# ykevinc/pocket-tts

Measured on AMD Instinct MI355X. Metric: audio-sec/wall-sec (RTF) per GPU at batch=32 + p50 first-chunk latency, higher is better.
Workload: dtype f32; 1 GPU; b6369a24 batch=32 concurrent 10 s utterances per GPU (125 frames, voice prompt 125 frames, 40 text tokens), lsd_decode_steps=1 (BASELINE configs[2]); global_batch=32, utterance_frames=125, jobs=37, prompt_frames=125, parallelism=replicas x1

## Files before the change

### pocket-tts_amd/csrc/engine.cpp

```cpp
#include "engine.h"

#include <hip/hip_ext.h>

#include <algorithm>
#include <array>
#include <cstdlib>
#include <cmath>
#include <cstring>
#include <mutex>

namespace ptts {

namespace {
std::mutex& voice_mu() {
  static std::mutex m;
  return m;
}

int pick_splits(int M, int N, int K) {
  const int tiles = ((N + 31) / 32) * ((M + 31) / 32);
  const int chunks = K / 32;
  int s = std::max(1, 768 / std::max(1, tiles));
  s = std::min(s, std::max(1, chunks / 4));
  return std::min(s, 16);
// ... 164 lines not shown
  vpre_ = (const float**)dalloc((sizeof(float*) * B + 3) / 4);
  vlen_ = (int*)dalloc(B);
  slot_voice_.assign(B, nullptr);
  drained_.assign(B, 1);
  codec_ok_.assign(B, 1);
  admit_call_.assign(B, -1);
  slot_lsd_.assign(B, 0);
  cancelled_.assign(B, 0);
  share_voice_ = probe_env("PTTS_NO_SHARED_VOICE") == nullptr;
  if (share_voice_) {
    fbm_.kv.pre = vpre_;
    fbm_.kv.pre_len = vlen_;
  }
#ifdef PTTS_PROBES
  if (probe_env("PTTS_STAMPS")) {
    stamp_ring_ = (unsigned long long*)dalloc((size_t)STAMP_CAP * 4);
    stamp_ctr_ = (unsigned*)dalloc(1);
  }
#endif
  if (probe_env("PTTS_BACK_WG_CAP")) back_cap_ = atoi(probe_env("PTTS_BACK_WG_CAP"));
  if (probe_env("PTTS_FRONT_PRIO")) set_front_prio(atoi(probe_env("PTTS_FRONT_PRIO")));
  if (probe_env("PTTS_BACK_PRIO")) set_back_prio(atoi(probe_env("PTTS_BACK_PRIO")));
  if (probe_env("PTTS_FRONT_SKIP")) set_front_skip(atoi(probe_env("PTTS_FRONT_SKIP")));
  ysilu_ = dalloc((size_t)lsd_ * B * FD);
  mods_ = dalloc((size_t)lsd_ * B * NADA);
  xf_ = dalloc((size_t)B * FD);
  hf_ = dalloc((size_t)B * FD);
  uf_ = dalloc((size_t)B * FD);
  PTTS_REQUIRE(hx_floats(B) * 4 < (1ull << 31), "flow-head hand-off regions exceed 2 GB (lsd_decode_steps too large)");
  hx_ = dalloc(hx_floats(B));
  fhm_ = dalloc((size_t)lsd_ * ((B + 15) / 16) * (FDEPTH + 1) * 2 * 16 * FD);
  PTTS_HIP(hipMemset(hx_, 0xFF, hx_floats(B) * 4));
  PTTS_HIP(hipDeviceSynchronize());
  hctr_ = (int*)dalloc(4 * ((B + 15) / 16) + 4);
  herr_ = (int*)dalloc(4);
  for (int i = 0, ch = MD / 2; i < 3; ++i, ch /= 2) trb_[i] = dalloc((size_t)RATIOS[i] * ch);
  temb_ =dalloc((size_t)temb_row0(lsd_ + 1) * FD);
  rope_ = dalloc((size_t)max_ctx_ * 64);
  temb_tmp_ = dalloc((size_t)2 * lsd_ * FD);

  for (int q = 0; q < NHB; ++q) {
    h_pcm_[q] = (float*)halloc(sizeof(float) * B * FRAME);
    h_meta_[q] = nfr_ > 1 && q < nhb_ ? h_pcmp_[q / nfr_] + (size_t)B * nfr_ * FRAME + (q % nfr_) * mstride
                                      : (float*)halloc(sizeof(float) * meta_floats_);
    memset(h_meta_[q], 0, sizeof(float) * meta_floats_);
  }
  h_err_ = (int*)halloc(sizeof(int));
  *h_err_ = 0;
  h_slots_ = (int*)halloc(sizeof(int) * B);
  h_st_ = (SlotState*)halloc(sizeof(SlotState) * B);
  h_idle_ = (SlotState*)halloc(sizeof(SlotState));
  *h_idle_ = SlotState{};
  h_idle_->eos_step = -1;
  h_fp_ = (int*)halloc(sizeof(int) * B);
  h_ids_ = (int*)halloc(sizeof(int) * PREFILL);
  h_tab_ = (int*)halloc(sizeof(int) * 4 * PREFILL);
  h_plat_ = (float*)halloc(sizeof(float) * PREFILL * LDIM);
  h_alat_ = (float*)halloc(sizeof(float) * B * LDIM);
  h_aopt_ = (int*)halloc(sizeof(int) * B);
  h_vpre_ = (const float**)halloc(sizeof(const float*) * B);
  h_vlen_ = (int*)halloc(sizeof(int) * B);
  memset(h_vpre_, 0, sizeof(float*) * B);
  memset(h_vlen_, 0, sizeof(int) * B);
  PTTS_HIP(hipStreamCreateWithFlags(&stream_be_, hipStreamNonBlocking));
  for (int q = 0; q < NHB; ++q) {
    PTTS_HIP(hipEventCreateWithFlags(&ev_front_[q], hipEventDisableTiming));
// ... 240 lines not shown
  auto it = split_.find(a.W);
  PTTS_REQUIRE(it != split_.end(), "bf16x6 tile without a split weight copy");
  a.Whm = it->second.first;
  a.Wlo = it->second.second;
}

void Engine::finalize() {
  PTTS_HIP(hipSetDevice(dev_));
  if (wq_ != QUANT_NONE && q8map_.empty()) derive_int8();
  if (fp8_ && f8map_.empty()) derive_fp8();
  if (gvmap_.empty()) derive_gemv();
  if (back_mfma_ == PTTS_BACK_F32X6 && split_.empty()) derive_split();
  if (!inw_t_) {
    void* p = nullptr;
    PTTS_HIP(hipMalloc(&p, sizeof(float) * LDIM * D));
    allocs_.push_back(p);
    inw_t_ = (float*)p;
  }
  transpose(W(L_.input_linear), D, LDIM, inw_t_, stream_);
  if (!fh_inw_t_) {
    void* p = nullptr;
    PTTS_HIP(hipMalloc(&p, sizeof(float) * LDIM * FD));
    allocs_.push_back(p);
    fh_inw_t_ = (float*)p;
  }
  transpose(W(L_.inproj_w), FD, LDIM, fh_inw_t_, stream_);
  if (!fhw_ && head_uniform_stride()) {
    void* p = nullptr;
    PTTS_HIP(hipMalloc(&p, sizeof(float) * flow_head_packed_floats()));
    allocs_.push_back(p);
    fhw_ = (float*)p;
  }
  if (fhw_) pack_flow_head(W(L_.rb_w0[0]), W(L_.rb_w2[0]), (long)(L_.rb_w0[1] - L_.rb_w0[0]), W(L_.fin_w), fhw_, stream_);
  TimeEmbedWeights tw;
  for (int i = 0; i < 2; ++i) {
    tw.l1w[i] = W(L_.te_l1w[i]);
    tw.l1b[i] = W(L_.te_l1b[i]);
    tw.l2w[i] = W(L_.te_l2w[i]);
    tw.l2b[i] = W(L_.te_l2b[i]);
    tw.alpha[i] = W(L_.te_alpha[i]);
  }
  for (int n = 1; n <= lsd_; ++n) time_embeddings(tw, n, temb_tmp_, temb_ + (size_t)temb_row0(n) * FD, stream_);
  rope_table(rope_, max_ctx_, stream_);
  for (int i = 0, ch = MD / 2; i < 3; ++i, ch /= 2)
    for (int p = 0; p < RATIOS[i]; ++p)
      PTTS_HIP(hipMemcpyAsync(trb_[i] + (size_t)p * ch, W(L_.dtr_b[i]), sizeof(float) * ch, hipMemcpyDeviceToDevice,
                              stream_));
  PTTS_HIP(hipGetLastError());
  PTTS_HIP(hipStreamSynchronize(stream_));
  ready_ = true;
}

void Engine::run_ops(const std::vector<Op>& ops) {
  xh_dirty_ = true;
  run_ops_on(ops, stream_);
}

void Engine::run_ops_on(const std::vector<Op>& ops, hipStream_t s) {
  for (const Op& op : ops) {
    op.fn(s);
    hipError_t e = hipGetLastError();
    if (e != hipSuccess) throw Error(PTTS_ERR_HIP, "launch of " + op.name + " failed: " + hipGetErrorString(e));
  }
}

void Engine::derive_int8() {
// ... 233 lines not shown
    const Layout::TL& t = L_.fl[l];
    const std::string p = tag + ".l" + std::to_string(l);
    KvStore kv = fb.kv;
    kv.base += (long)l * fb.kv_layer;
    if (kv.pre) kv.layer = l;
    int S = 1;
    linear_split(ops, p + ".qkv_gemm", fb.h, D, M, W(t.in_proj), 3 * D, D, &S, fb);
    if (step) {
      const float* P = fb.partial;
      float* O = fb.o;
      const float* rope = rope_;
      const double L = plan_ctx_ > 0 ? plan_ctx_ : max_ctx_ / 2.0;
      const double kvu = plan_kvu_ > 0 ? plan_kvu_ : M * L;
      ops.push_back({p + ".attention", [=](hipStream_t s) { attention_step_qkv(P, S, M, NH, map, kv, rope, O, s); },
                     (double)M * 4096.0 * L,
                     8192.0 * kvu + (double)M * (4.0 * (S * 3.0 * D + 2.0 * D + D) + 64.0 * 4 * 2)});
    } else {
      {
        const float* P = fb.partial;
        float* Q = fb.q;
        ops.push_back({p + ".qkv_rope", [=](hipStream_t s) { qkv_rope_append(P, S, nullptr, M, NH, map, kv, Q, s); }});
      }
      const float* Q = fb.q;
      float* O = fb.o;
      RowMap am = map;
      int Ma = M;
      if (map.ptab) {
        am.tab = map.ptab;
        Ma = map.mpad;
      }
      ops.push_back({p + ".attention", [=](hipStream_t s) { attention(Q, Ma, NH, am, kv, 0, O, s); }});
    }
    auto rr = [&](const std::string& name, int S2, int N, int act, bool resid, float* Y, const float* lnw,
                  const float* lnb, bool ln, float* Hout, float* Hfrag = nullptr) {
      RowReduceArgs a{};
      a.Hfrag = Hfrag;
      a.P = fb.partial;
      a.S = S2;
      a.M = M;
      a.N = N;
      a.act = act;
      if (resid) {
        a.R = fb.x;
        a.ldr = D;
      }
      a.Y = Y;
      a.ldy = N;
      a.ln = ln ? 1 : 0;
      a.ln_w = lnw;
      a.ln_b = lnb;
      a.eps = 1e-5f;
      a.Hout = Hout;
      a.ldh = N;
      push_rr(ops, name, a);
    };
    linear_split(ops, p + ".out_gemm", fb.o, D, M, W(t.out_proj), D, D, &S, fb);
    auto fk = step && gemv_fk_supported(M, FF, D) ? fkmap_.find(W(t.l1)) : fkmap_.end();
    const bool use_fk = fk != fkmap_.end() && hfrag_;
    rr(p + ".out_reduce_ln2", S, D, ACT_NONE, true, fb.x, W(t.n2w), W(t.n2b), true, fb.h, use_fk ? hfrag_ : nullptr);
    auto ffn = use_fk && ffn_hand_ ? ffnmap_.find(W(t.l2)) : ffnmap_.end();
    if (ffn != ffnmap_.end()) {
      static_assert(NL % 2 == 0, "the fused FFN's hand-off sets alternate by layer");
      const float *A = hfrag_, *P1 = fk->second, *P2 = ffn->second;
      float *hand = ffn_hand_, *Pp = fb.partial;
      int* err = herr_;
      const int set = l & 1;
      const int groups = ffn_groups_;
      auto f8 = ffn8map_.find(W(t.l2));
      const uint32_t *Q1 = nullptr, *Q2 = nullptr;
      const float *s1 = nullptr, *s2 = nullptr;
      if (f8 != ffn8map_.end()) {
        Q1 = f8->second.first.first;
        s1 = f8->second.first.second;
        Q2 = f8->second.second.first;
        s2 = f8->second.second.second;
      }
      const bool e4m3 = fp8_ && Q1;
      Op op{p + ".ffn", [=](hipStream_t s) { ffn_fused(A, M, P1, P2, groups, hand, set, Pp, err, s, Q1, s1, Q2, s2, e4m3); },
            2.0 * M * FF * D * 2,
            (Q1 ? 2.0 * FF * D + 8.0 * (FF + D) : 8.0 * FF * D) + 4.0 * ((double)M * D + (double)groups * M * D)};
      op.prep = [hand](hipStream_t s) { PTTS_HIP(hipMemsetD32Async(hand, 0xFFFFFFFFu, 2 * FFN_HAND_FLOATS, s)); };
      ops.push_back(op);
      S = groups;
    } else {
      if (use_fk) {
        const float* Pk = fk->second;
        const float* A = hfrag_;
        float* U = fb.u;
        ops.push_back({p + ".ff1_gemm", [=](hipStream_t s) { gemv_fk(A, M, FF, Pk, nullptr, ACT_GELU, U, FF, s); },
                       2.0 * M * FF * D, 4.0 * ((double)FF * D + (double)M * D + (double)M * FF)});
      } else {
        linear_split(ops, p + ".ff1_gemm", fb.h, D, M, W(t.l1), FF, D, &S, fb);
        rr(p + ".ff1_reduce_gelu", S, FF, ACT_GELU, false, fb.u, nullptr, nullptr, false, nullptr);
      }
      linear_split(ops, p + ".ff2_gemm", fb.u, FF, M, W(t.l2), D, FF, &S, fb);
    }
    if (l + 1 < NL)
      rr(p + ".ff2_reduce_ln1", S, D, ACT_NONE, true, fb.x, W(L_.fl[l + 1].n1w), W(L_.fl[l + 1].n1b), true, fb.h);
    else
      rr(p + ".ff2_reduce_outnorm", S, D, ACT_NONE, true, fb.x, W(L_.out_norm_w), W(L_.out_norm_b), out_norm, fb.h);
  }
}

void Engine::prefill_rows(std::vector<Op>& ops, int slot, int T, int p0, const FlowBufs& fb) {
  {
    float *x = fb.x, *h = fb.h;
    const float* w = W(L_.fl[0].n1w);
    const float* b = W(L_.fl[0].n1b);
    ops.push_back({"prefill.ln1", [=](hipStream_t s) { layernorm(x, D, h, D, T, D, w, b, 1e-5f, s); }});
  }
  RowMap map{slot, T, p0, nullptr};
  flow_layers(ops, T, map, false, false, "prefill", fb);
}

bool Engine::use_head_chain(int B) const {
  if (!flow_head_fits(B)) return false;
  if (flow_head_grid(B) > head_resident_) return false;
  return head_uniform_stride();
}

bool Engine::head_uniform_stride() const {
  const long s = (long)(L_.rb_w0[1] - L_.rb_w0[0]);
  for (int i = 1; i < FDEPTH; ++i)
    if ((long)(L_.rb_lnw[i] - L_.rb_lnw[i - 1]) != s || (long)(L_.rb_lnb[i] - L_.rb_lnb[i - 1]) != s ||
        (long)(L_.rb_w0[i] - L_.rb_w0[i - 1]) != s || (long)(L_.rb_b0[i] - L_.rb_b0[i - 1]) != s ||
        (long)(L_.rb_w2[i] - L_.rb_w2[i - 1]) != s || (long)(L_.rb_b2[i] - L_.rb_b2[i - 1]) != s)
      return false;
  return true;
}

void Engine::build_front(std::vector<Op>& ops, int B, int hb, int lsd_run) {
  PTTS_REQUIRE(lsd_run >= 1 && lsd_run <= lsd_, "lsd_run outside [1, cap]");
  int S = 1;
  const FlowBufs& fb = fbm_;
  flow_layers(ops, B, RowMap{0, 1, 0, fpos_}, true, true, "flow", fb);
  linear_split(ops, "head.cond_eos_gemm", fb.h, D, B, W(L_.cond_eos_w), NCOND, D, &S, fb);
  PTTS_REQUIRE(S <= FLOW_COND_MAX_SLABS, "head.flow_cond sums at most 16 split-K slabs");
  {
    const float* P = fb.partial;
    const float* bias = W(L_.cond_eos_b);
    const float* temb = temb_;
    const int lsd = lsd_run, cap = lsd_;
    SlotState* st = st_;
    float *ys = ysilu_, *cur = cur_, *eos = eos_;
    ops.push_back({"head.flow_cond", [=](hipStream_t s) { flow_cond(P, S, B, bias, temb, lsd, cap, st, ys, cur, eos, s); },
                   (double)B * NCOND * (S + 1) + 4.0 * lsd * B * FD,
                   4.0 * ((double)S * B * NCOND + NCOND + lsd * FD + lsd * (double)B * FD + B * (LDIM + 1.0))});
  }
  linear_split(ops, "head.ada_gemm", ysilu_, FD, lsd_run * B, W(L_.ada_w), NADA, FD, &S, fb);
  {
    RowReduceArgs a{};
    a.P = fb.partial;
    a.S = S;
    a.M = lsd_run * B;
    a.N = NADA;
    a.bias = W(L_.ada_b);
    a.Y = mods_;
    a.ldy = NADA;
    if (use_head_chain(B)) {
      const size_t r0 = (size_t)((B + 15) / 16 * 16) * FD;
      a.fill = hx_ + r0;
      a.fill_n4 = (long)((hx_floats(B, lsd_run) - r0) / 4);
      a.x0_cur = cur_;
      a.x0_w = fh_inw_t_;
      a.x0_b = W(L_.inproj_b);
      a.x0_hx = hx_;
      a.x0_B = B;
      a.fhm = fhm_;
      a.fhm_B = B;
    }
    push_rr(ops, "head.ada_reduce", a);
  }
  if (use_head_chain(B)) {
    FlowHeadArgs f{};
    f.B = B;
    f.lsd = lsd_run;
    f.st = st_;
    f.cur = cur_;
    f.mods = mods_;
    f.ldm = NADA;
    f.in_w = W(L_.inproj_w);
    f.in_b = W(L_.inproj_b);
    f.lnw = W(L_.rb_lnw[0]);
    f.lnb = W(L_.rb_lnb[0]);
    f.w0 = W(L_.rb_w0[0]);
    f.b0 = W(L_.rb_b0[0]);
    f.w2 = W(L_.rb_w2[0]);
    f.b2 = W(L_.rb_b2[0]);
    f.blk = (long)(L_.rb_w0[1] - L_.rb_w0[0]);
    f.fin_w = W(L_.fin_w);
    f.fin_b = W(L_.fin_b);
    f.wp = fhw_;
    f.fhm = fhm_;
    f.hx = hx_;
    f.x0_ready = 1;
    f.ctr = hctr_;
    f.err = herr_;
    f.dbg = probe_env("PTTS_HEAD_DBG") ? (unsigned long long*)strtoull(probe_env("PTTS_HEAD_DBG"), nullptr, 0) : nullptr;
    const double fl = 2.0 * lsd_run * B * ((double)FD * LDIM + 2.0 * FDEPTH * FD * FD + (double)LDIM * FD);
    const double by = 4.0 * ((double)FD * LDIM + 2.0 * FDEPTH * FD * FD + (double)LDIM * FD) +
                      4.0 * lsd_run * B * ((double)FDEPTH * 3 * FD + 2 * FD);
    float* hx = hx_;
    const size_t nhx = hx_floats(B, lsd_run);
    const float *cur = cur_, *iw = fh_inw_t_, *ib = W(L_.inproj_b);
// ... 2404 lines not shown
```

### pocket-tts_amd/csrc/engine.h

```cpp
#pragma once
#include <functional>
#include <map>
#include <string>
#include <vector>

#include "common.h"
#include "kernels.h"
#include "weights.h"

struct ptts_voice {
  int F = 0;
  float* kv = nullptr;
  std::vector<float> cond;
  const void* owner = nullptr;
  mutable int refs = 0;
  mutable bool dead = false;
  hipEvent_t ev = nullptr;
  float* h_cond = nullptr;
  mutable bool ordered = false;
};

namespace ptts {

struct VoicePlan;
// ... 175 lines not shown
  long ring_slot_ = 0, ring_layer_ = 0;
  int* fpos_ = nullptr;
  bool share_voice_ = true;
  const float** vpre_ = nullptr;
  int* vlen_ = nullptr;
  const float** h_vpre_ = nullptr;
  int* h_vlen_ = nullptr;
  std::vector<const ptts_voice*> slot_voice_;
  void voice_release(int slot, bool drained);
  SlotState* st_ = nullptr;
  float *lat_in_ = nullptr, *cur_ = nullptr, *eos_ = nullptr;
  int hist_T_[8] = {}, hist_C_[8] = {}, hist_P_[8] = {};

  static constexpr int PREFILL = 2048;
  static constexpr size_t TAIL_CAP = (size_t)16 << 20;
  static constexpr int TICKETS = 1024;
  int* ids_dev_ = nullptr;
  int* rowtab_dev_ = nullptr;
  int *ctab_dev_ = nullptr, *qrow_dev_ = nullptr, *orow_dev_ = nullptr;
  int* admit_slots_ = nullptr;
  SlotState* admit_st_ = nullptr;
  int* admit_fpos_ = nullptr;
  float *plat_dev_ = nullptr, *h_plat_ = nullptr, *admit_lat_ = nullptr, *h_alat_ = nullptr;
  int *admit_opt_ = nullptr, *h_aopt_ = nullptr;
  float *ysilu_ = nullptr, *mods_ = nullptr, *xf_ = nullptr, *hf_ = nullptr, *uf_ = nullptr;
  bool head_uniform_stride() const;
  bool use_head_chain(int B) const;
  float* fhw_ = nullptr;
  float* hx_ = nullptr;
  float* fhm_ = nullptr;
  float* fh_inw_t_ = nullptr;
  size_t hx_floats(int B) const { return hx_floats(B, lsd_); }
  size_t hx_floats(int B, int lsd) const { return (size_t)lsd * 13 * ((B + 15) / 16 * 16) * FD; }
  float* inw_t_ = nullptr;
  int *hctr_ = nullptr, *herr_ = nullptr;
  float* trb_[3] = {};
  static constexpr int NHB = NHB_MAX;
  int nhb_ = 3;
  int nfr_ = 1;
  int back_mfma_ = PTTS_BACK_F32;
  std::map<const float*, std::pair<const unsigned*, const unsigned short*>> split_;
  void derive_split();
  void attach_split(GemmArgs& a) const;
  int rows_hb_[NHB] = {};
  float* pcmp_[NHB / 2] = {};
  float* h_pcmp_[NHB / 2] = {};
  SlotState* h_act_ = nullptr;
  std::vector<int> act_slots_;
  int admit_delay_ = 0;
  double plan_ctx_ = 0, plan_win_ = 0, plan_kvu_ = 0;
  float* lat_out_[NHB] = {};
  float* eos_out_[NHB] = {};
  FrameFlags* flags_[NHB] = {};
  float* pcm_[NHB] = {};
  float* meta_[NHB] = {};
  size_t meta_floats_ = 0;
  int back_cap_ = 1;
  bool pipeline_ = false;
  hipStream_t stream_be_ = nullptr;
  hipEvent_t ev_front_[NHB] = {}, ev_back_[NHB] = {};
  hipEvent_t ev_admit_ = nullptr;
  hipEvent_t ev_be_tail_ = nullptr;
  hipEvent_t ev_act_ = nullptr;
  bool admit_pending_ = false;
  void mark_admission();
  long long k_ = 0;
// ... 125 lines not shown
```

### pocket-tts_amd/csrc/kernels.h

```cpp
#pragma once
#include <hip/hip_runtime.h>

#include <cstdint>
#include <vector>

namespace ptts {

enum Act : int { ACT_NONE = 0, ACT_GELU = 1, ACT_SILU = 2, ACT_ELU = 3 };

struct SlotState;
struct RowReduceArgs {
  const float* P;
  int S, M, N;
  const float* bias;
  int act;
  const float* gate;
  long ldg;
  const float* R;
  long ldr;
  float* Y;
  long ldy;
  float* Y2;
  float* euler;
  const SlotState* euler_st;
// ... 252 lines not shown
  float temp, eos_threshold, noise_clamp;
  unsigned long long seed;
  int lsd;
};
struct FrameFlags {
  int valid;
  int last;
};

constexpr int FLOW_COND_MAX_SLABS = 16;
constexpr int temb_row0(int n) { return n * (n - 1) / 2; }
void flow_cond(const float* P, int S, int B, const float* bias, const float* temb, int lsd_run, int lsd_cap,
               const SlotState* st, float* ysilu, float* cur, float* eos_out, hipStream_t s);

constexpr int FH_D = 512, FH_L = 32, FH_DEPTH = 6;
struct FlowHeadArgs {
  int B, lsd;
  const SlotState* st;
  float* cur;
  const float* mods;
  long ldm;
  const float *in_w, *in_b;
  const float *lnw, *lnb, *w0, *b0, *w2, *b2;
  long blk;
  const float *fin_w, *fin_b;
  const float* wp;
  const float* fhm;
  float* hx;
  int x0_ready;
  int* ctr;
  int* err;
  unsigned long long* dbg;
};
void set_wg_cap(int cap);
void set_back_hi(int on);
#ifdef PTTS_PROBES
constexpr unsigned STAMP_CAP = 1u << 16;
void stamp(unsigned long long* ring, unsigned* ctr, unsigned tag, hipStream_t s);
#endif
void set_front_prio(int prio);
void set_back_prio(int prio);
void set_front_skip(int v);
bool flow_head_fits(int B);
void flow_head_x0(const float* cur, const float* w_t, const float* bias, float* hx, int B, hipStream_t s);
size_t flow_head_packed_floats();
void pack_flow_head(const float* w0, const float* w2, long blk, const float* fin_w, float* dst, hipStream_t s);
int flow_head_grid(int B);
int flow_head_max_resident(int dev);
void input_ln(const float* lat, const float* Wt, const float* lnw, const float* lnb, float* x, float* h, int M,
              hipStream_t s);
void transpose(const float* src, int rows, int cols, float* dst, hipStream_t s);
void flow_head(const FlowHeadArgs& a, hipStream_t s);

struct FrontCommitArgs {
  int B;
  SlotState* st;
  const float* eos;
  const float* cur;
  float* lat_in;
  float* lat_out;
  float* eos_out;
  FrameFlags* flags;
  int* fpos;
  const float *Wt, *lnw, *lnb;
  float *x, *h;
  const int* err_dev;
// ... 198 lines not shown
```

### pocket-tts_amd/csrc/kernels.hip

```cpp
#include "kernels.h"

#include <cmath>
#include <stdexcept>

#include "devfn.h"

namespace ptts {

#ifdef PTTS_PROBES
#define PTTS_PROBE(a) ((a).probe)
#else
#define PTTS_PROBE(a) 0
#endif

static thread_local int g_wg_cap = 0;
void set_wg_cap(int cap) { g_wg_cap = cap; }
static thread_local int g_back_hi = 1;
void set_back_hi(int on) { g_back_hi = on; }
#ifdef PTTS_PROBES
__device__ int g_front_prio = 0;
void set_front_prio(int prio) {
  if (hipMemcpyToSymbol(HIP_SYMBOL(g_front_prio), &prio, sizeof prio) != hipSuccess)
    throw std::runtime_error("set_front_prio failed");
}
// ... 1788 lines not shown
  }
  PTTS_GEMV(4, 128)
  PTTS_GEMV(2, 64)
  PTTS_GEMV(1, 64)
  PTTS_GEMV(1, 32)
#undef PTTS_GEMV
}


__device__ __forceinline__ float act1(float x, int act) {
  return act == ACT_GELU ? gelu_tanh(x) : (act == ACT_SILU ? silu(x) : (act == ACT_ELU ? elu1(x) : x));
}

template <int SMAX>
__device__ __forceinline__ float4 rr_value(const RowReduceArgs& a, int m, int n) {
  const float* p = a.P + (long)m * a.N + n;
  const long zs = (long)a.M * a.N;
  float4 pz[SMAX];
#pragma unroll
  for (int z = 0; z < SMAX; ++z) pz[z] = *reinterpret_cast<const float4*>(p + (long)min(z, a.S - 1) * zs);
  const float4 bi = *reinterpret_cast<const float4*>((a.bias ? a.bias + n : p));
  const float4 ga = *reinterpret_cast<const float4*>((a.gate ? a.gate + (long)m * a.ldg + n : p));
  const float4 rr = *reinterpret_cast<const float4*>((a.R ? a.R + (long)m * a.ldr + n : p));
  float4 v = pz[0];
#pragma unroll
  for (int z = 1; z < SMAX; ++z)
    if (z < a.S) v = f4add(v, pz[z]);
  if (a.bias) v = f4add(v, bi);
  if (a.act != ACT_NONE) v = make_float4(act1(v.x, a.act), act1(v.y, a.act), act1(v.z, a.act), act1(v.w, a.act));
  if (a.gate) v = f4mul(v, ga);
  if (a.R) v = f4add(v, rr);
  return v;
}
__device__ __forceinline__ void rr_store(const RowReduceArgs& a, int m, int n, float4 v) {
  if (a.Y) *reinterpret_cast<float4*>(a.Y + (long)m * a.ldy + n) = v;
  if (a.fhm) {
    const int st = m / a.fhm_B, b = m - st * a.fhm_B, RG = (a.fhm_B + 15) / 16;
    const int i = min(n / (3 * FH_D), FH_DEPTH), rem = n - i * 3 * FH_D;
    const int t = rem / FH_D, k = rem - t * FH_D;
    if (t < 2) {
      const long idx = (((((long)(st * RG + b / 16) * (FH_DEPTH + 1) + i) * 2 + t) * 8 + (k >> 6)) * 4 + ((k >> 4) & 3)) * 64 +
                       (b & 15) + 16 * ((k >> 2) & 3);
      reinterpret_cast<float4*>(a.fhm)[idx] = v;
    }
  }
  if (a.Y2) *reinterpret_cast<float4*>(a.Y2 + (long)m * a.ldy + n) = make_float4(elu1(v.x), elu1(v.y), elu1(v.z), elu1(v.w));
  if (a.euler) {
    float4* e = reinterpret_cast<float4*>(a.euler + (long)m * 32 + n);
    const int nr = max(a.euler_st[m].lsd, 1);
    const float sc = 1.0f / (float)nr;
    const float4 c = *e;
    const float4 nx = make_float4(c.x + v.x * sc, c.y + v.y * sc, c.z + v.z * sc, c.w + v.w * sc);
    *e = a.euler_step < nr ? nx : c;
  }
}
__device__ __forceinline__ float4 rr_ln(const RowReduceArgs& a, int m, int n, float4 d, float den) {
  float4 hh = make_float4(d.x / den, d.y / den, d.z / den, d.w / den);
  if (a.ln_w)
    hh = f4add(f4mul(hh, *reinterpret_cast<const float4*>(a.ln_w + n)), *reinterpret_cast<const float4*>(a.ln_b + n));
  if (a.mshift) {
    const float4 sc = *reinterpret_cast<const float4*>(a.mscale + (long)m * a.ldm + n);
    const float4 sf = *reinterpret_cast<const float4*>(a.mshift + (long)m * a.ldm + n);
    hh = make_float4(hh.x * (1.0f + sc.x) + sf.x, hh.y * (1.0f + sc.y) + sf.y, hh.z * (1.0f + sc.z) + sf.z,
                     hh.w * (1.0f + sc.w) + sf.w);
  }
  return hh;
}

__device__ __forceinline__ float fh_dot4(float4 c, float4 w) { return (c.x * w.x + c.y * w.y) + (c.z * w.z + c.w * w.w); }
__device__ __forceinline__ float4 fh_inproj4(const float4 (&cv)[8], const float* in_w, const float* in_b, int n) {
  float acc[4];
#pragma unroll
  for (int q = 0; q < 4; ++q) {
    const float* w = in_w + (long)(n + q) * FH_L;
    float t = in_b[n + q];
#pragma unroll
    for (int j = 0; j < 8; ++j) t += fh_dot4(cv[j], *reinterpret_cast<const float4*>(w + 4 * j));
    acc[q] = t;
  }
  return make_float4(acc[0], acc[1], acc[2], acc[3]);
}

__device__ __forceinline__ void fh_x0_job(const float* cur, const float* w_t, const float* bias, float* hx, int B,
                                          long i0, long nthr) {
  for (long i = i0; i < (long)B * FH_D; i += nthr) {
    const int b = (int)(i / FH_D), n = (int)(i % FH_D);
    float t = bias[n];
#pragma unroll
    for (int j = 0; j < 8; ++j) {
      const float4 c = *reinterpret_cast<const float4*>(cur + (long)b * FH_L + 4 * j);
      const float* w = w_t + (long)(4 * j) * FH_D + n;
      t += fh_dot4(c, make_float4(w[0], w[FH_D], w[2 * FH_D], w[3 * FH_D]));
    }
    if (t != t) t = __uint_as_float(0x7FC00000u);
    hx[((long)((b >> 4) * 32 + (n >> 4))) * 256 + (b & 15) * 16 + (n & 15)] = t;
  }
}
__global__ void k_fh_x0(const float* cur, const float* w, const float* bias, float* hx, int B) {
  fh_x0_job(cur, w, bias, hx, B, (long)blockIdx.x * 256 + threadIdx.x, (long)gridDim.x * 256);
}
void flow_head_x0(const float* cur, const float* w_t, const float* bias, float* hx, int B, hipStream_t s) {
  hipLaunchKernelGGL(k_fh_x0, dim3((B * FH_D + 255) / 256), dim3(256), 0, s, cur, w_t, bias, hx, B);
}

template <int SMAX>
__global__ __launch_bounds__(256) void k_row_reduce(RowReduceArgs a) {
  if (a.front) front_prio();
  __shared__ float sh[4];
  if (a.fill) {
    const long nthr = (long)gridDim.x * gridDim.y * 256;
    for (long i = ((long)blockIdx.y * gridDim.x + blockIdx.x) * 256 + threadIdx.x; i < a.fill_n4; i += nthr)
      reinterpret_cast<uint4*>(a.fill)[i] = make_uint4(~0u, ~0u, ~0u, ~0u);
  }
  if (a.x0_hx)
    fh_x0_job(a.x0_cur, a.x0_w, a.x0_b, a.x0_hx, a.x0_B, ((long)blockIdx.y * gridDim.x + blockIdx.x) * 256 + threadIdx.x,
              (long)gridDim.x * gridDim.y * 256);
  const int m = blockIdx.x;
  const int n0 = blockIdx.y * 1024 + 4 * threadIdx.x;
  const bool ok = n0 < a.N;
  const int n = ok ? n0 : 0;
  const float4 v = rr_value<SMAX>(a, m, n);
  if (ok) rr_store(a, m, n, v);
  if (!a.ln) return;
  const float s = ok ? (v.x + v.y) + (v.z + v.w) : 0.f;
  const float mean = block_sum(s, sh) / (float)a.N;
  const float4 d = make_float4(v.x - mean, v.y - mean, v.z - mean, v.w - mean);
  const float q = ok ? (d.x * d.x + d.y * d.y) + (d.z * d.z + d.w * d.w) : 0.f;
  const float den = sqrtf(block_sum(q, sh) / (float)a.N + a.eps);
// ... 470 lines not shown
void attention16_qkv(const float* qkv, int M, int nh, RowMap map, KvStore kv, int window, float* O, hipStream_t s) {
  if (map.tab != nullptr || map.rps != 16) throw std::runtime_error("attention16_qkv: needs 16 rows per slot");
  if ((kv.cap & (kv.cap - 1)) != 0 || kv.cap < window + 16)
    throw std::runtime_error("attention16_qkv: ring too small for the fused append");
  const dim3 grid((M + 15) / 16, nh);
  hipLaunchKernelGGL((k_attn16<true, true>), grid, dim3(64 * A16_WAVES), cap_lds(k_attn16<true, true>, g_wg_cap), s,
                     qkv, M, nh, map, kv, window, O);
}

void attention(const float* Q, int M, int nh, RowMap map, KvStore kv, int window, float* O, hipStream_t s) {
  if (kv.pre != nullptr && window > 0)
    throw std::runtime_error("attention: shared voice prefixes need the 16-row causal kernel");
  const dim3 grid((M + 15) / 16, nh);
  if ((kv.cap & (kv.cap - 1)) == 0)
    hipLaunchKernelGGL(k_attn16<true>, grid, dim3(64 * A16_WAVES), cap_lds(k_attn16<true>, g_wg_cap), s, Q, M, nh, map, kv, window, O);
  else
    hipLaunchKernelGGL(k_attn16<false>, grid, dim3(64 * A16_WAVES), cap_lds(k_attn16<false>, g_wg_cap), s, Q, M, nh, map, kv, window, O);
}

__device__ __forceinline__ unsigned long long mix64(unsigned long long z) {
  z = (z ^ (z >> 30)) * 0xBF58476D1CE4E5B9ull;
  z = (z ^ (z >> 27)) * 0x94D049BB133111EBull;
  return z ^ (z >> 31);
}
__device__ float normal_at(unsigned long long seed, int step, int k, int attempt) {
  const unsigned long long base =
      mix64(seed * 0x9E3779B97F4A7C15ull + (unsigned long long)step * 0xD1B54A32D192ED03ull +
            (unsigned long long)(k * 64 + attempt) * 0x8CB92BA72F3D8DD7ull);
  const float u1 = ((float)(base >> 41) + 0.5f) * (1.0f / 8388608.0f);
  const float u2 = (float)(mix64(base ^ 0x5851F42D4C957F2Dull) >> 40) * (1.0f / 16777216.0f);
  return sqrtf(-2.0f * logf(u1)) * cosf(6.283185307179586f * u2);
}

__global__ __launch_bounds__(256) void k_flow_cond(const float* P, int S, int B, const float* bias, const float* temb,
                                                   int lsd, int lsd_cap, const SlotState* st, float* ysilu,
                                                   float* cur, float* eos_out) {
  front_prio();
  const int b = blockIdx.x, tid = threadIdx.x;
  const int NC = 513;
  const long zs = (long)B * NC;
  const float* p0 = P + (long)b * NC + tid;
  float v0[16], v1[16], ve[16];
#pragma unroll
  for (int z = 0; z < 16; ++z) {
    v0[z] = z < S ? p0[z * zs] : 0.f;
    v1[z] = z < S ? p0[z * zs + 256] : 0.f;
    ve[z] = (z < S && tid == 0) ? P[(long)b * NC + 512 + z * zs] : 0.f;
  }
  const SlotState& ss = st[b];
  const float temp = ss.temp, clamp = ss.noise_clamp;
  const unsigned long long seed = ss.seed;
  const int step = ss.step;
  const int nrow = min(max(ss.lsd, 1), lsd_cap);
  const float* tn = temb + (long)temb_row0(nrow) * 512;
  const float b0 = bias[tid], b1 = bias[tid + 256], be = bias[512];
  float c0 = 0.f, c1 = 0.f, e = 0.f;
#pragma unroll
  for (int z = 0; z < 16; ++z)
    if (z < S) {
      c0 += v0[z];
      c1 += v1[z];
      e += ve[z];
    }
  c0 += b0;
  c1 += b1;
  for (int s = 0; s < lsd; ++s) {
    const int ts = min(s, nrow - 1);
    ysilu[((long)s * B + b) * 512 + tid] = silu(tn[ts * 512 + tid] + c0);
    ysilu[((long)s * B + b) * 512 + tid + 256] = silu(tn[ts * 512 + tid + 256] + c1);
  }
  if (tid == 0) eos_out[b] = e + be;
  if (tid < 32) {
    float x0 = 0.f;
    if (temp > 0.f) {
      const float sd = sqrtf(temp);
      x0 = sd * normal_at(seed, step, tid, 0);
      if (clamp > 0.f) {
        int att = 1;
        while (fabsf(x0) > clamp && att < 64) x0 = sd * normal_at(seed, step, tid, att++);
        x0 = fminf(fmaxf(x0, -clamp), clamp);
      }
    }
    cur[b * 32 + tid] = x0;
  }
}

void flow_cond(const float* P, int S, int B, const float* bias, const float* temb, int lsd_run, int lsd_cap,
               const SlotState* st, float* ysilu, float* cur, float* eos_out, hipStream_t s) {
  if (S < 1 || S > FLOW_COND_MAX_SLABS) throw std::runtime_error("flow_cond: 1..16 split-K slabs");
  if (lsd_run < 1 || lsd_run > lsd_cap) throw std::runtime_error("flow_cond: lsd_run outside [1, cap]");
  hipLaunchKernelGGL(k_flow_cond, dim3(B), dim3(256), 0, s, P, S, B, bias, temb, lsd_run, lsd_cap, st, ysilu, cur,
                     eos_out);
}

struct QuantUpArgs {
  const float* latent[NFR_MAX];
  const FrameFlags* fl[NFR_MAX];
  int nfr;
  const float *emb_std, *emb_mean, *wq, *wup, *qprev_in;
  float* qprev_out;
  float *x, *h;
  const float *ln_w, *ln_b;
};
__global__ __launch_bounds__(256) void k_quant_upsample(QuantUpArgs a) {
  __shared__ float sz[NFR_MAX][32];
  __shared__ float sx[4 * 512];
  const int b = blockIdx.x, f = blockIdx.y >> 2, r0 = (blockIdx.y & 3) * 4, tid = threadIdx.x;
  const int T = 16 * a.nfr;
  float4 wqr[2][8], wur[2][2];
  float qpv[2];
#pragma unroll
  for (int u = 0; u < 2; ++u) {
    const int c = tid + 256 * u;
#pragma unroll
    for (int i = 0; i < 8; ++i) wqr[u][i] = *reinterpret_cast<const float4*>(a.wq + c * 32 + 4 * i);
    wur[u][0] = *reinterpret_cast<const float4*>(a.wup + c * 32 + r0);
    wur[u][1] = *reinterpret_cast<const float4*>(a.wup + c * 32 + 16 + r0);
    qpv[u] = a.qprev_in[(long)b * 512 + c];
  }
  if (tid < 32 * a.nfr) {
    const int g = tid >> 5, k = tid & 31;
    sz[g][k] = a.latent[g][b * 32 + k] * a.emb_std[k] + a.emb_mean[k];
  }
  __syncthreads();
#pragma unroll
// ... 1741 lines not shown
```

Baseline: 5227 audio-sec/wall-sec.

## Fuse flow-head cond/eos GEMM, flow_cond, ada GEMM and reduce into one prelude kernel

Replaces the four-launch head sequence (cond_eos split-K GEMM, flow_cond, ada split-K GEMM, ada reduce) with a single producer/consumer kernel. Producer blocks compute the cond/eos product with MFMA from the hfrag layout and publish silu'd conditioning tiles through a sentinel-filled hand-off buffer. Consumer blocks preload packed ada weights, spin on those tiles, and write mods and the fhm layout directly, also generating noise and x0 and filling hx. The aim is to cut launch and partial-sum traffic on the per-frame critical path, at the cost of spin-wait coupling, an extra memset prep, and reliance on every block being co-resident.

```diff
diff --git a/pocket-tts_amd/csrc/engine.cpp b/pocket-tts_amd/csrc/engine.cpp
--- a/pocket-tts_amd/csrc/engine.cpp
+++ b/pocket-tts_amd/csrc/engine.cpp
@@ -220,6 +220,7 @@
   fhm_ = dalloc((size_t)lsd_ * ((B + 15) / 16) * (FDEPTH + 1) * 2 * 16 * FD);
   PTTS_HIP(hipMemset(hx_, 0xFF, hx_floats(B) * 4));
   PTTS_HIP(hipDeviceSynchronize());
+  hp_hand_ = dalloc((size_t)lsd_ * 2 * HP_REGION_FLOATS);
   hctr_ = (int*)dalloc(4 * ((B + 15) / 16) + 4);
   herr_ = (int*)dalloc(4);
   for (int i = 0, ch = MD / 2; i < 3; ++i, ch /= 2) trb_[i] = dalloc((size_t)RATIOS[i] * ch);
@@ -526,6 +527,17 @@
     fhw_ = (float*)p;
   }
   if (fhw_) pack_flow_head(W(L_.rb_w0[0]), W(L_.rb_w2[0]), (long)(L_.rb_w0[1] - L_.rb_w0[0]), W(L_.fin_w), fhw_, stream_);
+  static_assert(HP_NCOND == NCOND_PAD && HP_NADA == NADA, "head_prelude's shapes are the flow head's");
+  if (wq_ == QUANT_NONE && !fp8_ && hfrag_ && gemv_fk_supported(1, NCOND_PAD, D)) {
+    if (!hp_w_) {
+      void* p = nullptr;
+      PTTS_HIP(hipMalloc(&p, sizeof(float) * ((size_t)NCOND_PAD * D + (size_t)NADA * FD)));
+      allocs_.push_back(p);
+      hp_w_ = (float*)p;
+    }
+    pack_gemv_fk(W(L_.cond_eos_w), NCOND_PAD, D, hp_w_, stream_);
+    pack_head_ada(W(L_.ada_w), hp_w_ + (size_t)NCOND_PAD * D, stream_);
+  }
   TimeEmbedWeights tw;
   for (int i = 0; i < 2; ++i) {
     tw.l1w[i] = W(L_.te_l1w[i]);
@@ -825,9 +837,12 @@
       ops.push_back({p + ".attention", [=](hipStream_t s) { attention(Q, Ma, NH, am, kv, 0, O, s); }});
     }
     auto rr = [&](const std::string& name, int S2, int N, int act, bool resid, float* Y, const float* lnw,
-                  const float* lnb, bool ln, float* Hout, float* Hfrag = nullptr) {
+                  const float* lnb, bool ln, float* Hout, float* Hfrag = nullptr, float* fill = nullptr,
+                  long fill_n4 = 0) {
       RowReduceArgs a{};
       a.Hfrag = Hfrag;
+      a.fill = fill;
+      a.fill_n4 = fill_n4;
       a.P = fb.partial;
       a.S = S2;
       a.M = M;
@@ -890,8 +905,12 @@
     }
     if (l + 1 < NL)
       rr(p + ".ff2_reduce_ln1", S, D, ACT_NONE, true, fb.x, W(L_.fl[l + 1].n1w), W(L_.fl[l + 1].n1b), true, fb.h);
-    else
-      rr(p + ".ff2_reduce_outnorm", S, D, ACT_NONE, true, fb.x, W(L_.out_norm_w), W(L_.out_norm_b), out_norm, fb.h);
+    else {
+      const bool pre = step && out_norm && use_head_prelude(M);
+      const long n4 = (long)lsd_ * ((M + 15) / 16) * HP_REGION_FLOATS / 4;
+      rr(p + ".ff2_reduce_outnorm", S, D, ACT_NONE, true, fb.x, W(L_.out_norm_w), W(L_.out_norm_b), out_norm, fb.h,
+         pre ? hfrag_ : nullptr, pre ? hp_hand_ : nullptr, pre ? n4 : 0);
+    }
   }
 }
 
@@ -910,6 +929,10 @@
   if (!flow_head_fits(B)) return false;
   if (flow_head_grid(B) > head_resident_) return false;
   return head_uniform_stride();
+}
+
+bool Engine::use_head_prelude(int B) const {
+  return hp_w_ && head_prelude_supported(B, 1) && gemv_fk_supported(B, NCOND_PAD, D) && use_head_chain(B);
 }
 
 bool Engine::head_uniform_stride() const {
@@ -927,42 +950,80 @@
   int S = 1;
   const FlowBufs& fb = fbm_;
   flow_layers(ops, B, RowMap{0, 1, 0, fpos_}, true, true, "flow", fb);
-  linear_split(ops, "head.cond_eos_gemm", fb.h, D, B, W(L_.cond_eos_w), NCOND, D, &S, fb);
-  PTTS_REQUIRE(S <= FLOW_COND_MAX_SLABS, "head.flow_cond sums at most 16 split-K slabs");
-  {
-    const float* P = fb.partial;
-    const float* bias = W(L_.cond_eos_b);
-    const float* temb = temb_;
-    const int lsd = lsd_run, cap = lsd_;
-    SlotState* st = st_;
-    float *ys = ysilu_, *cur = cur_, *eos = eos_;
-    ops.push_back({"head.flow_cond", [=](hipStream_t s) { flow_cond(P, S, B, bias, temb, lsd, cap, st, ys, cur, eos, s); },
-                   (double)B * NCOND * (S + 1) + 4.0 * lsd * B * FD,
-                   4.0 * ((double)S * B * NCOND + NCOND + lsd * FD + lsd * (double)B * FD + B * (LDIM + 1.0))});
-  }
-  linear_split(ops, "head.ada_gemm", ysilu_, FD, lsd_run * B, W(L_.ada_w), NADA, FD, &S, fb);
-  {
-    RowReduceArgs a{};
-    a.P = fb.partial;
-    a.S = S;
-    a.M = lsd_run * B;
-    a.N = NADA;
-    a.bias = W(L_.ada_b);
-    a.Y = mods_;
-    a.ldy = NADA;
-    if (use_head_chain(B)) {
-      const size_t r0 = (size_t)((B + 15) / 16 * 16) * FD;
-      a.fill = hx_ + r0;
-      a.fill_n4 = (long)((hx_floats(B, lsd_run) - r0) / 4);
-      a.x0_cur = cur_;
-      a.x0_w = fh_inw_t_;
-      a.x0_b = W(L_.inproj_b);
-      a.x0_hx = hx_;
-      a.x0_B = B;
-      a.fhm = fhm_;
-      a.fhm_B = B;
-    }
-    push_rr(ops, "head.ada_reduce", a);
+  if (use_head_prelude(B)) {
+    const int RG = (B + 15) / 16;
+    const size_t r0 = (size_t)(RG * 16) * FD;
+    HeadPreludeArgs a{};
+    a.B = B;
+    a.lsd = lsd_run;
+    a.lsd_cap = lsd_;
+    a.A = hfrag_;
+    a.Pc = hp_w_;
+    a.cbias = W(L_.cond_eos_b);
+    a.temb = temb_;
+    a.st = st_;
+    a.eos_out = eos_;
+    a.cur = cur_;
+    a.hand = hp_hand_;
+    a.Pa = hp_w_ + (size_t)NCOND_PAD * D;
+    a.abias = W(L_.ada_b);
+    a.mods = mods_;
+    a.fhm = fhm_;
+    a.x0_w = fh_inw_t_;
+    a.x0_b = W(L_.inproj_b);
+    a.x0_hx = hx_;
+    a.fill = hx_ + r0;
+    a.fill_n4 = (long)((hx_floats(B, lsd_run) - r0) / 4);
+    a.err = herr_;
+    const double mn = (double)lsd_run * B * NADA, hand = (double)lsd_run * RG * HP_REGION_FLOATS;
+    Op op{"head.prelude", [a](hipStream_t s) { head_prelude(a, s); },
+          2.0 * B * NCOND_PAD * D + 2.0 * lsd_run * B * NADA * FD + 2.0 * B * LDIM * FD + 4.0 * lsd_run * B * FD,
+          4.0 * ((double)NCOND_PAD * D + NCOND_PAD + (double)FK_A_FLOATS + (double)NADA * FD + NADA + lsd_run * FD +
+                 B * (LDIM + 1.0) + 2.0 * hand + mn + mn * 2.0 / 3.0 + (double)B * (LDIM + FD) + (double)LDIM * FD +
+                 4.0 * a.fill_n4)};
+    float* hh = hp_hand_;
+    const size_t nh = (size_t)lsd_run * RG * HP_REGION_FLOATS;
+    op.prep = [hh, nh](hipStream_t s) { PTTS_HIP(hipMemsetD32Async(hh, 0xFFFFFFFFu, nh, s)); };
+    ops.push_back(op);
+  } else {
+    linear_split(ops, "head.cond_eos_gemm", fb.h, D, B, W(L_.cond_eos_w), NCOND, D, &S, fb);
+    PTTS_REQUIRE(S <= FLOW_COND_MAX_SLABS, "head.flow_cond sums at most 16 split-K slabs");
+    {
+      const float* P = fb.partial;
+      const float* bias = W(L_.cond_eos_b);
+      const float* temb = temb_;
+      const int lsd = lsd_run, cap = lsd_;
+      SlotState* st = st_;
+      float *ys = ysilu_, *cur = cur_, *eos = eos_;
+      ops.push_back(
+          {"head.flow_cond", [=](hipStream_t s) { flow_cond(P, S, B, bias, temb, lsd, cap, st, ys, cur, eos, s); },
+           (double)B * NCOND * (S + 1) + 4.0 * lsd * B * FD,
+           4.0 * ((double)S * B * NCOND + NCOND + lsd * FD + lsd * (double)B * FD + B * (LDIM + 1.0))});
+    }
+    linear_split(ops, "head.ada_gemm", ysilu_, FD, lsd_run * B, W(L_.ada_w), NADA, FD, &S, fb);
+    {
+      RowReduceArgs a{};
+      a.P = fb.partial;
+      a.S = S;
+      a.M = lsd_run * B;
+      a.N = NADA;
+      a.bias = W(L_.ada_b);
+      a.Y = mods_;
+      a.ldy = NADA;
+      if (use_head_chain(B)) {
+        const size_t r0 = (size_t)((B + 15) / 16 * 16) * FD;
+        a.fill = hx_ + r0;
+        a.fill_n4 = (long)((hx_floats(B, lsd_run) - r0) / 4);
+        a.x0_cur = cur_;
+        a.x0_w = fh_inw_t_;
+        a.x0_b = W(L_.inproj_b);
+        a.x0_hx = hx_;
+        a.x0_B = B;
+        a.fhm = fhm_;
+        a.fhm_B = B;
+      }
+      push_rr(ops, "head.ada_reduce", a);
+    }
   }
   if (use_head_chain(B)) {
     FlowHeadArgs f{};
diff --git a/pocket-tts_amd/csrc/engine.h b/pocket-tts_amd/csrc/engine.h
--- a/pocket-tts_amd/csrc/engine.h
+++ b/pocket-tts_amd/csrc/engine.h
@@ -231,6 +231,8 @@
   float* fh_inw_t_ = nullptr;
   size_t hx_floats(int B) const { return hx_floats(B, lsd_); }
   size_t hx_floats(int B, int lsd) const { return (size_t)lsd * 13 * ((B + 15) / 16 * 16) * FD; }
+  bool use_head_prelude(int B) const;
+  float *hp_w_ = nullptr, *hp_hand_ = nullptr;
   float* inw_t_ = nullptr;
   int *hctr_ = nullptr, *herr_ = nullptr;
   float* trb_[3] = {};
diff --git a/pocket-tts_amd/csrc/kernels.h b/pocket-tts_amd/csrc/kernels.h
--- a/pocket-tts_amd/csrc/kernels.h
+++ b/pocket-tts_amd/csrc/kernels.h
@@ -308,6 +308,25 @@
   int* err;
   unsigned long long* dbg;
 };
+constexpr int HP_NCOND = 544, HP_NADA = (FH_DEPTH * 3 + 2) * FH_D;
+constexpr int HP_PRODUCERS = HP_NCOND / 16, HP_CONSUMERS = HP_NADA / 64;
+constexpr long HP_REGION_FLOATS = 16L * FH_D;
+struct HeadPreludeArgs {
+  int B, lsd, lsd_cap;
+  const float *A, *Pc, *cbias, *temb;
+  const SlotState* st;
+  float *eos_out, *cur, *hand;
+  const float *Pa, *abias;
+  float *mods, *fhm;
+  const float *x0_w, *x0_b;
+  float* x0_hx;
+  float* fill;
+  long fill_n4;
+  int* err;
+};
+bool head_prelude_supported(int B, int lsd_run);
+void pack_head_ada(const float* W, float* packed, hipStream_t s);
+void head_prelude(const HeadPreludeArgs& a, hipStream_t s);
 void set_wg_cap(int cap);
 void set_back_hi(int on);
 #ifdef PTTS_PROBES
diff --git a/pocket-tts_amd/csrc/kernels.hip b/pocket-tts_amd/csrc/kernels.hip
--- a/pocket-tts_amd/csrc/kernels.hip
+++ b/pocket-tts_amd/csrc/kernels.hip
@@ -1844,17 +1844,20 @@
   if (a.R) v = f4add(v, rr);
   return v;
 }
+__device__ __forceinline__ long fhm_index(int st, int b, int B, int n) {
+  const int RG = (B + 15) / 16;
+  const int i = min(n / (3 * FH_D), FH_DEPTH), rem = n - i * 3 * FH_D;
+  const int t = rem / FH_D, k = rem - t * FH_D;
+  if (t >= 2) return -1;
+  return (((((long)(st * RG + b / 16) * (FH_DEPTH + 1) + i) * 2 + t) * 8 + (k >> 6)) * 4 + ((k >> 4) & 3)) * 64 +
+         (b & 15) + 16 * ((k >> 2) & 3);
+}
 __device__ __forceinline__ void rr_store(const RowReduceArgs& a, int m, int n, float4 v) {
   if (a.Y) *reinterpret_cast<float4*>(a.Y + (long)m * a.ldy + n) = v;
   if (a.fhm) {
-    const int st = m / a.fhm_B, b = m - st * a.fhm_B, RG = (a.fhm_B + 15) / 16;
-    const int i = min(n / (3 * FH_D), FH_DEPTH), rem = n - i * 3 * FH_D;
-    const int t = rem / FH_D, k = rem - t * FH_D;
-    if (t < 2) {
-      const long idx = (((((long)(st * RG + b / 16) * (FH_DEPTH + 1) + i) * 2 + t) * 8 + (k >> 6)) * 4 + ((k >> 4) & 3)) * 64 +
-                       (b & 15) + 16 * ((k >> 2) & 3);
-      reinterpret_cast<float4*>(a.fhm)[idx] = v;
-    }
+    const int st = m / a.fhm_B;
+    const long idx = fhm_index(st, m - st * a.fhm_B, a.fhm_B, n);
+    if (idx >= 0) reinterpret_cast<float4*>(a.fhm)[idx] = v;
   }
   if (a.Y2) *reinterpret_cast<float4*>(a.Y2 + (long)m * a.ldy + n) = make_float4(elu1(v.x), elu1(v.y), elu1(v.z), elu1(v.w));
   if (a.euler) {
@@ -1893,19 +1896,23 @@
   return make_float4(acc[0], acc[1], acc[2], acc[3]);
 }
 
+__device__ __forceinline__ void fh_x0_one(const float* c, const float* w_t, const float* bias, float* hx, int b,
+                                          int n) {
+  float t = bias[n];
+#pragma unroll
+  for (int j = 0; j < 8; ++j) {
+    const float4 cj = *reinterpret_cast<const float4*>(c + 4 * j);
+    const float* w = w_t + (long)(4 * j) * FH_D + n;
+    t += fh_dot4(cj, make_float4(w[0], w[FH_D], w[2 * FH_D], w[3 * FH_D]));
+  }
+  if (t != t) t = __uint_as_float(0x7FC00000u);
+  hx[((long)((b >> 4) * 32 + (n >> 4))) * 256 + (b & 15) * 16 + (n & 15)] = t;
+}
 __device__ __forceinline__ void fh_x0_job(const float* cur, const float* w_t, const float* bias, float* hx, int B,
                                           long i0, long nthr) {
   for (long i = i0; i < (long)B * FH_D; i += nthr) {
     const int b = (int)(i / FH_D), n = (int)(i % FH_D);
-    float t = bias[n];
-#pragma unroll
-    for (int j = 0; j < 8; ++j) {
-      const float4 c = *reinterpret_cast<const float4*>(cur + (long)b * FH_L + 4 * j);
-      const float* w = w_t + (long)(4 * j) * FH_D + n;
-      t += fh_dot4(c, make_float4(w[0], w[FH_D], w[2 * FH_D], w[3 * FH_D]));
-    }
-    if (t != t) t = __uint_as_float(0x7FC00000u);
-    hx[((long)((b >> 4) * 32 + (n >> 4))) * 256 + (b & 15) * 16 + (n & 15)] = t;
+    fh_x0_one(cur + (long)b * FH_L, w_t, bias, hx, b, n);
   }
 }
 __global__ void k_fh_x0(const float* cur, const float* w, const float* bias, float* hx, int B) {
@@ -2442,6 +2449,20 @@
   return sqrtf(-2.0f * logf(u1)) * cosf(6.283185307179586f * u2);
 }
 
+__device__ __forceinline__ float flow_noise(float temp, float clamp, unsigned long long seed, int step, int k) {
+  float x0 = 0.f;
+  if (temp > 0.f) {
+    const float sd = sqrtf(temp);
+    x0 = sd * normal_at(seed, step, k, 0);
+    if (clamp > 0.f) {
+      int att = 1;
+      while (fabsf(x0) > clamp && att < 64) x0 = sd * normal_at(seed, step, k, att++);
+      x0 = fminf(fmaxf(x0, -clamp), clamp);
+    }
+  }
+  return x0;
+}
+
 __global__ __launch_bounds__(256) void k_flow_cond(const float* P, int S, int B, const float* bias, const float* temb,
                                                    int lsd, int lsd_cap, const SlotState* st, float* ysilu,
                                                    float* cur, float* eos_out) {
@@ -2480,19 +2501,7 @@
     ysilu[((long)s * B + b) * 512 + tid + 256] = silu(tn[ts * 512 + tid + 256] + c1);
   }
   if (tid == 0) eos_out[b] = e + be;
-  if (tid < 32) {
-    float x0 = 0.f;
-    if (temp > 0.f) {
-      const float sd = sqrtf(temp);
-      x0 = sd * normal_at(seed, step, tid, 0);
-      if (clamp > 0.f) {
-        int att = 1;
-        while (fabsf(x0) > clamp && att < 64) x0 = sd * normal_at(seed, step, tid, att++);
-        x0 = fminf(fmaxf(x0, -clamp), clamp);
-      }
-    }
-    cur[b * 32 + tid] = x0;
-  }
+  if (tid < 32) cur[b * 32 + tid] = flow_noise(temp, clamp, seed, step, tid);
 }
 
 void flow_cond(const float* P, int S, int B, const float* bias, const float* temb, int lsd_run, int lsd_cap,
@@ -2501,6 +2510,174 @@
   if (lsd_run < 1 || lsd_run > lsd_cap) throw std::runtime_error("flow_cond: lsd_run outside [1, cap]");
   hipLaunchKernelGGL(k_flow_cond, dim3(B), dim3(256), 0, s, P, S, B, bias, temb, lsd_run, lsd_cap, st, ysilu, cur,
                      eos_out);
+}
+
+__global__ void k_pack_head_ada(const float* __restrict__ W, float* __restrict__ P) {
+  const long i4 = (long)blockIdx.x * 256 + threadIdx.x;
+  if (i4 >= (long)HP_NADA * FH_D / 4) return;
+  const int l = (int)(i4 & 63), j = (int)((i4 >> 6) & 7), c2 = (int)((i4 >> 9) & 1), w = (int)((i4 >> 10) & 7);
+  const int cw = (int)(i4 >> 13);
+  const int n = 64 * cw + 32 * (w >> 2) + 16 * c2 + (l & 15), k = 128 * (w & 3) + 32 * (l >> 4) + 4 * j;
+  reinterpret_cast<float4*>(P)[i4] = *reinterpret_cast<const float4*>(W + (long)n * FH_D + k);
+}
+void pack_head_ada(const float* W, float* packed, hipStream_t s) {
+  hipLaunchKernelGGL(k_pack_head_ada, dim3(HP_NADA * FH_D / 4 / 256), dim3(256), 0, s, W, packed);
+}
+
+__global__ __launch_bounds__(512) void k_head_prelude(HeadPreludeArgs a) {
+  front_prio();
+  __shared__ __attribute__((aligned(16))) float red[8 * 2 * 4 * 64];
+  __shared__ __attribute__((aligned(16))) float sC[32 * 16];
+  const int tid = threadIdx.x, lane = tid & 63;
+  const int w = __builtin_amdgcn_readfirstlane(tid >> 6);
+  const int RG = (a.B + 15) >> 4;
+  typedef float f4v __attribute__((ext_vector_type(4)));
+  const auto hr = sc1_rsrc(a.hand);
+  if (blockIdx.x < HP_PRODUCERS) {
+    const int ct = blockIdx.x;
+    const f4v* wp = reinterpret_cast<const f4v*>(a.Pc) + ((long)(ct * 8 + w) * 8) * 64 + lane;
+    const f4v* ap = reinterpret_cast<const f4v*>(a.A) + ((long)(w * 2) * 8) * 64 + lane;
+    f4v b[8], a0[8], a1[8];
+#pragma unroll
+    for (int j = 0; j < 8; ++j)
+      b[j] = (front_skip() & 1) ? f4v{0.f, 0.f, 0.f, 0.f} : __builtin_nontemporal_load(wp + j * 64);
+#pragma unroll
+    for (int j = 0; j < 8; ++j) {
+      a0[j] = ap[j * 64];
+      a1[j] = ap[(8 + j) * 64];
+    }
+    __builtin_amdgcn_sched_barrier(0);
+    floatx4 c0 = {0.f, 0.f, 0.f, 0.f}, c1 = {0.f, 0.f, 0.f, 0.f};
+#pragma unroll
+    for (int j = 0; j < 8; ++j) {
+      if (front_skip() & 2) break;
+#pragma unroll
+      for (int e = 0; e < 4; ++e) {
+        c0 = __builtin_amdgcn_mfma_f32_16x16x4f32(a0[j][e], b[j][e], c0, 0, 0, 0);
+        c1 = __builtin_amdgcn_mfma_f32_16x16x4f32(a1[j][e], b[j][e], c1, 0, 0, 0);
+      }
+    }
+#pragma unroll
+    for (int i = 0; i < 4; ++i) {
+      red[((w * 2 + 0) * 4 + i) * 64 + lane] = c0[i];
+      red[((w * 2 + 1) * 4 + i) * 64 + lane] = c1[i];
+    }
+    __syncthreads();
+    {
+      const int t = tid >> 8, i = (tid >> 6) & 3, ll = tid & 63;
+      float v = red[((0 * 2 + t) * 4 + i) * 64 + ll];
+#pragma unroll
+      for (int ww = 1; ww < 8; ++ww) v += red[((ww * 2 + t) * 4 + i) * 64 + ll];
+      const int row = 16 * t + (ll >> 4) * 4 + i, col = ct * 16 + (ll & 15);
+      v += a.cbias[col];
+      if (col == FH_D && row < a.B) a.eos_out[row] = v;
+      sC[row * 16 + (ll & 15)] = v;
+    }
+    __syncthreads();
+    if (ct < FH_D / 16 && tid < 128) {
+      const int m = tid & 31, c4 = tid >> 5, k = 16 * ct + 4 * c4;
+      if ((m >> 4) < RG) {
+        const bool live = m < a.B;
+        const float4 c = *reinterpret_cast<const float4*>(&sC[m * 16 + 4 * c4]);
+        const int nrow = live ? min(max(a.st[m].lsd, 1), a.lsd_cap) : 1;
+        const float* tn = a.temb + (long)temb_row0(nrow) * FH_D + k;
+        const int off = (((k >> 7) * 8 + ((k >> 2) & 7)) * 64 + ((k >> 5) & 3) * 16 + (m & 15)) * 16;
+        for (int s = 0; s < a.lsd; ++s) {
+          const float4 te = *reinterpret_cast<const float4*>(tn + (long)min(s, nrow - 1) * FH_D);
+          float4 y = make_float4(silu(te.x + c.x), silu(te.y + c.y), silu(te.z + c.z), silu(te.w + c.w));
+          if (!live) y = make_float4(0.f, 0.f, 0.f, 0.f);
+          fh_put(hr, (s * RG + (m >> 4)) * (int)(HP_REGION_FLOATS * 4) + off, y);
+        }
+      }
+    }
+    return;
+  }
+  const int cw = blockIdx.x - HP_PRODUCERS;
+  const int kq = w & 3;
+  const f4v* wp = reinterpret_cast<const f4v*>(a.Pa) + ((long)((cw * 8 + w) * 2) * 8) * 64 + lane;
+  f4v b0[8], b1[8];
+#pragma unroll
+  for (int j = 0; j < 8; ++j) {
+    b0[j] = (front_skip() & 1) ? f4v{0.f, 0.f, 0.f, 0.f} : __builtin_nontemporal_load(wp + j * 64);
+    b1[j] = (front_skip() & 1) ? f4v{0.f, 0.f, 0.f, 0.f} : __builtin_nontemporal_load(wp + (8 + j) * 64);
+  }
+  __builtin_amdgcn_sched_barrier(0);
+  if (cw < 4 * a.B) {
+    const int b = cw >> 2, q = cw & 3;
+    if (tid < FH_L) {
+      const SlotState& ss = a.st[b];
+      const float x0 = flow_noise(ss.temp, ss.noise_clamp, ss.seed, ss.step, tid);
+      sC[tid] = x0;
+      if (q == 0) a.cur[b * FH_L + tid] = x0;
+    }
+    __syncthreads();
+    if (tid < 128) fh_x0_one(sC, a.x0_w, a.x0_b, a.x0_hx, b, 128 * q + tid);
+  }
+  for (long i = (long)cw * 512 + tid; i < a.fill_n4; i += (long)HP_CONSUMERS * 512)
+    reinterpret_cast<uint4*>(a.fill)[i] = make_uint4(~0u, ~0u, ~0u, ~0u);
+  bool dead = false;
+  for (int s = 0; s < a.lsd; ++s)
+    for (int t = 0; t < RG; ++t) {
+      const int aoff = (s * RG + t) * (int)(HP_REGION_FLOATS * 4) + (kq * 8 * 64 + lane) * 16;
+      float4 av[8];
+#pragma unroll
+      for (int j = 0; j < 8; ++j) av[j] = fh_ld(hr, aoff + j * 64 * 16);
+      unsigned spins = 0;
+      while (!dead) {
+        bool ok = true;
+#pragma unroll
+        for (int j = 0; j < 8; ++j) ok &= !fh_empty(av[j]);
+        if (__all(ok)) break;
+        __builtin_amdgcn_s_sleep(1);
+#pragma unroll
+        for (int j = 0; j < 8; ++j)
+          if (fh_empty(av[j])) av[j] = fh_ld(hr, aoff + j * 64 * 16);
+        if (++spins > (1u << 20)) {
+          if (lane == 0) __hip_atomic_store(a.err, 1, __ATOMIC_RELAXED, __HIP_MEMORY_SCOPE_AGENT);
+          dead = true;
+        }
+      }
+      floatx4 c0 = {0.f, 0.f, 0.f, 0.f}, c1 = {0.f, 0.f, 0.f, 0.f};
+#pragma unroll
+      for (int j = 0; j < 8; ++j) {
+        if (front_skip() & 2) break;
+        const float ae[4] = {av[j].x, av[j].y, av[j].z, av[j].w};
+#pragma unroll
+        for (int e = 0; e < 4; ++e) {
+          c0 = __builtin_amdgcn_mfma_f32_16x16x4f32(ae[e], b0[j][e], c0, 0, 0, 0);
+          c1 = __builtin_amdgcn_mfma_f32_16x16x4f32(ae[e], b1[j][e], c1, 0, 0, 0);
+        }
+      }
+      __syncthreads();
+#pragma unroll
+      for (int i = 0; i < 4; ++i) {
+        red[((w * 2 + 0) * 4 + i) * 64 + lane] = c0[i];
+        red[((w * 2 + 1) * 4 + i) * 64 + lane] = c1[i];
+      }
+      __syncthreads();
+      if (tid < 256) {
+        const int ctl = tid >> 6, r = (tid >> 2) & 15, q4 = tid & 3;
+        const float* rp = red + (((ctl >> 1) * 4 * 2 + (ctl & 1)) * 4 + (r & 3)) * 64 + (r >> 2) * 16 + 4 * q4;
+        float4 v = *reinterpret_cast<const float4*>(rp);
+#pragma unroll
+        for (int kk = 1; kk < 4; ++kk) v = f4add(v, *reinterpret_cast<const float4*>(rp + kk * 2 * 4 * 64));
+        const int brow = 16 * t + r, n = 64 * cw + 16 * ctl + 4 * q4;
+        if (brow < a.B) {
+          v = f4add(v, *reinterpret_cast<const float4*>(a.abias + n));
+          *reinterpret_cast<float4*>(a.mods + ((long)s * a.B + brow) * HP_NADA + n) = v;
+          const long idx = fhm_index(s, brow, a.B, n);
+          if (idx >= 0) reinterpret_cast<float4*>(a.fhm)[idx] = v;
+        }
+      }
+    }
+}
+
+bool head_prelude_supported(int B, int lsd_run) { return B >= 1 && B <= 32 && lsd_run >= 1; }
+
+void head_prelude(const HeadPreludeArgs& a, hipStream_t s) {
+  if (!head_prelude_supported(a.B, a.lsd) || a.lsd > a.lsd_cap) throw std::runtime_error("head_prelude: bad shape");
+  hipLaunchKernelGGL(k_head_prelude, dim3(HP_PRODUCERS + HP_CONSUMERS), dim3(512), cap_lds(k_head_prelude, g_wg_cap), s,
+                     a);
 }
 
 struct QuantUpArgs {
```

After: 5325 audio-sec/wall-sec, median of 6. 1.9% higher.
